# Liupeter01/Software-Rasterizer

Measured on AMD Instinct MI355X. Metric: frames_per_sec, higher is better.
Workload: dtype f32

## Files before the change

### software-rasterizer_amd/csrc/srz_api.hip

```cpp
#include <dlfcn.h>

#include <algorithm>
#include <cmath>
#include <cstdio>
#include <cstdlib>
#include <cstring>
#include <new>
#include <string>
#include <vector>

#include "srz_device.h"

using namespace srz;

namespace {
std::string g_create_error;

struct EventPair {
  hipEvent_t t0, t1, t2, t3;
  bool detailed;
};

struct BatchDesc {
  int32_t shader, tex_id;
// ... 88 lines not shown
  uint32_t *d_sparse_rows = nullptr;
  uint32_t *d_slow_list = nullptr, *d_slow_count = nullptr;
  uint4 *d_redo_list = nullptr;
  uint32_t fast_kinds = 0;
  bool any_generic = true;
  uint32_t *d_vis = nullptr, *d_work_count = nullptr, *d_chunk_rows = nullptr;
  uint4 *d_worklist = nullptr;
  uint64_t kind_slots = 0;
  uint32_t kind_mask = 0, n_kind_slots = 0;
  bool approx_shade = false;
  bool no_packed = false;
  uint32_t *d_band_desc = nullptr;
  uint2 *d_band_ent = nullptr;
  uint64_t total_groups = 0;
  ShadeDescG *d_sdesc = nullptr;
  DrawDesc *d_draws = nullptr;
  static constexpr int STAGE_RING = 4;
  uint8_t *d_dyn = nullptr;
  size_t dyn_bytes = 0, dyn_lights_off = 0, dyn_draws_off = 0;
  uint8_t *h_stage[STAGE_RING] = {};
  hipEvent_t stage_ev[STAGE_RING] = {};
  bool stage_busy[STAGE_RING] = {};
  unsigned stage_next = 0;
  std::vector<DrawDesc> h_draws;
  std::vector<int> h_draw_mesh;
  uint32_t n_draws = 0, max_faces = 0;
  uint64_t sdesc_version = 0;
  uint32_t tiles_x = 0, max_tiles = 0;
  bool have_stats = false;
  bool update_failed = false;
  static constexpr int CLEAR_TUNE_SKIP = 6, CLEAR_TUNE_AGAIN = 4096;
  struct ClearTune {
    uint32_t wgs = CLEAR_GRID_DEFAULT;
    bool done = false;
    int renders = 0;
    int since = 0;
    ClearCtl *d_ctl = nullptr;
    uint32_t *h_wgs = nullptr;
  } clear_tune;
  srz_stats stats{};
};

namespace {

hipStream_t pick_stream(const srz_ctx *ctx, void *stream) {
  if (!stream) return ctx->stream;
// ... 303 lines not shown
  if (!ct.done && ct.renders == 0)
    if (const uint32_t m = clear_memo(ctx, fs, 0u)) ct.wgs = p.wgs = m, ct.done = true;
  if (ct.done) return SRZ_OK;
  const uint32_t h = *static_cast<volatile uint32_t *>(ct.h_wgs);
  const int j = ct.renders - srz_frameset::CLEAR_TUNE_SKIP;
  if (h != 0u) {
    ct.wgs = p.wgs = h, ct.done = true;
    clear_memo(ctx, fs, h);
  } else if (!detailed && j < 0) {
    p.count = true;
  } else if (!detailed) {
    p.wgs = CLEAR_GRID_MAX, p.dev_wgs = &ct.d_ctl->wgs;
    p.count = p.stamp = j < CLEAR_TUNE_RENDERS;
  }
  return SRZ_OK;
}

void end_clear_plan(srz_frameset *fs, const ClearPlan &p, hipStream_t s) {
  if (p.count) ++fs->clear_tune.renders;
  if (p.stamp) launch_clear_tune(fs->clear_tune.d_ctl, fs->clear_tune.h_wgs, s);
  if (p.rebase) launch_clear_rebase(fs->clear_tune.d_ctl, s);
}

struct RenderPlan {
  Pass pass;
  hipStream_t s;
  bool side, turns, vertex_setup;
  ClearPlan clear;
  EventPair *ep;
};

int enqueue_sub_batch(srz_ctx *ctx, srz_frameset *fs, const RenderPlan &r, RenderArgs &a, int f0, int n, int part) {
  const bool stats = r.pass.kind == Pass::COUNTING;
  const hipStream_t s = r.s;
  const size_t tpf = (size_t)fs->n_local_bands * fs->tiles_x;
  RenderArgs v = a;
  if (n != fs->n_frames) {
    const int fa = r.pass.f_begin + f0;
    v.frames += fa, v.n_frames = (uint32_t)n;
    v.vis += (size_t)fa * tpf * ((size_t)TILE * TILE);
    v.tile_info += (size_t)fa * tpf;
    v.out += (size_t)fa * a.frame_stride;
    v.work_cap = (uint32_t)((size_t)(n < 8 ? n : (n + 7) / 8) * tpf);
  }
  const uint32_t tiles = (uint32_t)((size_t)n * tpf);
  if (r.vertex_setup) launch_chunks(v, n, fs->max_tris, s);
  else launch_setup(v, n, fs->max_tris, stats, s);
  launch_bin(v, n, fs->max_tris, s);
  if (!fs->pool_sized && !stats) {
    HIP_TRY(ctx, copy_demand(fs, part, s));
    HIP_TRY(ctx, hipStreamSynchronize(s));
    const uint32_t need = max_pool_demand(fs, part, part + 1);
    if (need > fs->pool_sub_cap) {
      if (int rc = grow_pool(ctx, fs, need, 8u)) return rc;
      a.pool = v.pool = fs->d_pool, a.pool_sub_cap = v.pool_sub_cap = fs->pool_sub_cap;
      HIP_TRY(ctx, hipMemsetAsync(fs->d_pool_heads, 0, sizeof(uint32_t) * CNT_STRIDE * fs->pool_n_sub, s));
      launch_bin(v, n, fs->max_tris, s);
    }
  }
  if (r.pass.kind == Pass::SIZE_ONLY) return SRZ_OK;
  if (r.ep) HIP_TRY(ctx, hipEventRecord(r.ep->t1, s));
  const unsigned ev = r.side ? ctx->ev_next++ % srz_ctx::EV_RING : 0u;
  if (r.side) {
    HIP_TRY(ctx, hipEventRecord(ctx->ev_fork[ev], s));
    HIP_TRY(ctx, hipStreamWaitEvent(ctx->stream2, ctx->ev_fork[ev], 0));
    launch_clear(v, tiles, ctx->stream2, r.clear.wgs);
    HIP_TRY(ctx, copy_demand(fs, part, ctx->stream2));
    HIP_TRY(ctx, hipEventRecord(ctx->ev_join[ev], ctx->stream2));
  }
// ... 26 lines not shown
  const uint32_t need = max_pool_demand(fs, 0, srz_frameset::DEMAND_PARTS);
  if (need > fs->pool_sub_cap)
    if (int rc = grow_pool(ctx, fs, need, 4u)) return rc;
  RenderArgs a = make_args(ctx, fs, d_out, flags_or, pass);
  if (!size_only) fs->last_flags = flags_or, fs->rendered = true;
  EventPair ep{};
  const bool timed = ctx->timing != 0 && !stats && !size_only && ctx->ev_used.size() < 65536, detailed = timed && ctx->timing >= 2;
  if (timed)
    if (int rc = begin_timing(ctx, ep, detailed, s)) return rc;
  if (stats) HIP_TRY(ctx, hipMemsetAsync(ctx->d_stats, 0, ST_COUNT * sizeof(unsigned long long), s));
  if (fs->max_tris == 0) {
    HIP_TRY(ctx, hipMemsetAsync(fs->d_work_count, 0, sizeof(uint32_t) * CNT_STRIDE * N_WORK_LISTS, s));
    HIP_TRY(ctx, hipMemsetAsync(fs->d_pool_heads, 0, sizeof(uint32_t) * CNT_STRIDE * fs->pool_n_sub, s));
    HIP_TRY(ctx, hipMemsetAsync(fs->d_slow_count, 0, 2 * sizeof(uint32_t), s));
  }
  const bool turns = !stats && !size_only && fs->max_tiles >= 8192;
  if (turns && !ctx->ev_raster[0])
    if (int rc = create_side(ctx, "render: raster events", nullptr, false, ctx->ev_raster)) return rc;
  if (turns && ctx->raster_valid && ctx->raster_last_stream != s) {
    HIP_TRY(ctx, hipStreamWaitEvent(s, ctx->ev_raster[(ctx->raster_next + srz_ctx::EV_RING - 1) % srz_ctx::EV_RING], 0));
    a.other_streams = 1u;
  }
  const bool vertex_setup = fs->d_draws != nullptr && !stats;
  if (fs->d_draws) launch_vertex(fs->d_draws, fs->n_draws, fs->max_faces, fs->d_tris, fs->d_tri_pos, fs->d_frames, vertex_setup ? fs->d_bbox : nullptr, s);
  const bool any_fused = any_frame_has(fs, flags_or, SRZ_FUSED_CLEAR), side = any_fused && fs->max_tiles >= 8192 && !size_only;
  if (side && !ctx->stream2)
    if (int rc = create_side(ctx, "render: clear stream", &ctx->stream2, true, ctx->ev_fork, ctx->ev_join)) return rc;
  if (!side && any_fused) a.clear_in_raster = 1u;
  RenderPlan r{pass, s, side, turns, vertex_setup, ClearPlan{}, detailed ? &ep : nullptr};
  if (side)
    if (int rc = plan_clear(ctx, fs, pass, detailed, s, r.clear)) return rc;
  a.clear_wgs_dev = r.clear.dev_wgs;
  const int n_all = pass.f_count < 0 ? fs->n_frames : pass.f_count;
  const int chunk = sub_batch_frames(ctx, fs, n_all, stats || detailed);
  for (int f0 = 0, part = 0; f0 < n_all; f0 += chunk, ++part)
    if (int rc = enqueue_sub_batch(ctx, fs, r, a, f0, std::min(chunk, n_all - f0), part)) return rc;
  if (!stats) fs->pool_sized = true;
  end_clear_plan(fs, r.clear, s);
  if (timed) {
    HIP_TRY(ctx, hipEventRecord(ep.t3, s));
    ctx->ev_used.push_back(ep);
  }
  HIP_TRY(ctx, hipGetLastError());
  return SRZ_OK;
}

int render_entry(const char *name, srz_ctx *ctx, srz_frameset *fs, void *d_out, size_t out_bytes, uint32_t flags, void *stream, Pass pass) {
  if (!ctx) return SRZ_E_INVALID;
  const std::string fn(name);
  if (!fs || !d_out) return fail(ctx, SRZ_E_INVALID, fn + ": null frameset / output");
  if (out_bytes < srz_frameset_out_bytes(ctx, fs)) return fail(ctx, SRZ_E_INVALID, fn + ": output buffer too small");
  if (((uintptr_t)d_out & 15u) != 0) return fail(ctx, SRZ_E_INVALID, fn + ": output must be 16-byte aligned");
// ... 130 lines not shown
  if (e != hipSuccess) {
    (void)hipFree(d_px);
    return fail(ctx, SRZ_E_NODEVICE, std::string("srz_texture_upload: ") + hipGetErrorString(e));
  }
  (void)hipFree(ctx->d_texmem[tex_id]);
  ctx->d_texmem[tex_id] = d_px;
  ctx->h_tex[tex_id] = TexDesc{d_px, w, h};
  ctx->tex_version++;
  return SRZ_OK;
}

static void set_shading(FrameDesc &d, const srz_frame &fr) {
  std::memcpy(d.eye, fr.eye, sizeof d.eye), std::memcpy(d.ka, fr.ka, sizeof d.ka), std::memcpy(d.ks, fr.ks, sizeof d.ks);
  d.p = fr.p, d.kh = fr.kh, d.kn = fr.kn;
  d.flags = fr.flags & FRAME_FLAGS;
}

static void stage_dyn(const srz_frameset *fs, uint8_t *st) {
  std::memcpy(st, fs->h_frames.data(), sizeof(FrameDesc) * fs->h_frames.size());
  if (!fs->h_lights.empty()) std::memcpy(st + fs->dyn_lights_off, fs->h_lights.data(), sizeof(srz_light) * fs->h_lights.size());
  if (!fs->h_draws.empty()) std::memcpy(st + fs->dyn_draws_off, fs->h_draws.data(), sizeof(DrawDesc) * fs->h_draws.size());
}

static int ensure_stage_ring(srz_ctx *ctx, srz_frameset *fs, const char *who) {
  if (fs->h_stage[0]) return SRZ_OK;
  for (int i = 0; i < srz_frameset::STAGE_RING; ++i) {
    hipError_t e = hipHostMalloc((void **)&fs->h_stage[i], fs->dyn_bytes, hipHostMallocDefault);
    if (e == hipSuccess) e = hipEventCreateWithFlags(&fs->stage_ev[i], hipEventDisableTiming);
    if (e != hipSuccess) {
      for (int j = 0; j <= i; ++j) {
        if (fs->h_stage[j]) (void)hipHostFree(fs->h_stage[j]);
        if (fs->stage_ev[j]) (void)hipEventDestroy(fs->stage_ev[j]);
        fs->h_stage[j] = nullptr, fs->stage_ev[j] = nullptr;
      }
      return fail(ctx, e == hipErrorOutOfMemory ? SRZ_E_NOMEM : SRZ_E_NODEVICE, std::string(who) + ": staging buffers: " + hipGetErrorString(e));
    }
  }
  return SRZ_OK;
}

static int upload_dyn(srz_ctx *ctx, srz_frameset *fs) {
  const unsigned slot = fs->stage_next++ % srz_frameset::STAGE_RING;
  if (fs->stage_busy[slot]) HIP_TRY(ctx, hipEventSynchronize(fs->stage_ev[slot]));
  stage_dyn(fs, fs->h_stage[slot]);
  HIP_TRY(ctx, hipMemcpyAsync(fs->d_dyn, fs->h_stage[slot], fs->dyn_bytes, hipMemcpyHostToDevice, ctx->stream));
  HIP_TRY(ctx, hipEventRecord(fs->stage_ev[slot], ctx->stream));
  fs->stage_busy[slot] = true;
  return SRZ_OK;
}

static int build_frameset(srz_ctx *ctx, const srz_frame *frames, int n_frames, srz_frameset **out, bool copy_tris, bool tris_aos = false,
                          const std::vector<DrawDesc> *draws = nullptr) {
  if (!ctx) return SRZ_E_INVALID;
  if (!out) return fail(ctx, SRZ_E_INVALID, "srz_frameset_create: out is NULL");
  *out = nullptr;
  if (!frames || n_frames <= 0) return fail(ctx, SRZ_E_INVALID, "srz_frameset_create: no frames");
  const int W = frames[0].width, H = frames[0].height;
  if (W <= 0 || H <= 0 || W > 32767 || H > 32767) return fail(ctx, SRZ_E_INVALID, "srz_frameset_create: width/height must be in 1..32767");
  HIP_TRY(ctx, hipSetDevice(ctx->device));
  srz_frameset *fs = new (std::nothrow) srz_frameset();
  if (!fs) return fail(ctx, SRZ_E_NOMEM, "srz_frameset_create: out of host memory");
  fs->n_frames = n_frames, fs->width = W, fs->height = H;
  fs->shard_rank = ctx->shard_rank, fs->shard_world = ctx->shard_world;
  shard_layout(H, fs->shard_rank, fs->shard_world, fs->n_bands, fs->n_local_bands, fs->bands_per_rank, fs->local_rows);
  fs->tiles_x = (uint32_t)((W + TILE - 1) / TILE);
  if ((uint64_t)((n_frames + 7) / 8 * 8) * fs->n_local_bands * fs->tiles_x >= 0x7fffffffull) {
    delete fs;
    return fail(ctx, SRZ_E_INVALID, "srz_frameset_create: frames x tiles exceeds the launch grid limit; split the batch");
  }
  uint64_t tri_off = 0, light_off = 0, batch_off = 0, group_off = 0;
  for (int f = 0; f < n_frames; ++f) {
    const srz_frame &fr = frames[f];
// ... 42 lines not shown
    const FrameDesc &d = fs->h_frames[f];
    size_t o = d.tri_off;
    for (uint32_t b = 0; b < fr.n_batches; ++b) {
      const srz_batch &sb = fr.batches[b];
      if (copy_tris && sb.n_tris) {
        std::memcpy(&h_tris[o], sb.tris, sizeof(srz_tri) * sb.n_tris);
        if (!h_pos.empty())
          for (size_t t = 0; t < sb.n_tris; ++t) std::memcpy(&h_pos[(o + t) * TRI_POS_F], &sb.tris[t].pos[0][0], sizeof(float) * TRI_POS_F);
      }
      std::fill(h_tb.begin() + o, h_tb.begin() + o + sb.n_tris, (uint16_t)b);
      o += sb.n_tris;
    }
    if (fr.n_lights) std::memcpy(&fs->h_lights[d.light_off], fr.lights, sizeof(srz_light) * fr.n_lights);
  }
  classify_frames(fs);
  if (draws) {
    fs->h_draws = *draws, fs->n_draws = (uint32_t)draws->size();
    for (const DrawDesc &dd : *draws) fs->max_faces = std::max(fs->max_faces, dd.n_faces);
  }
  auto up16 = [](size_t v) { return (v + 15) & ~(size_t)15; };
  fs->dyn_lights_off = up16(sizeof(FrameDesc) * (size_t)n_frames);
  fs->dyn_draws_off = up16(fs->dyn_lights_off + sizeof(srz_light) * (size_t)light_off);
  fs->dyn_bytes = fs->dyn_draws_off + sizeof(DrawDesc) * fs->h_draws.size();
  auto dev_alloc = [&](void **p, size_t bytes) { return hipMalloc(p, std::max<size_t>(bytes, 256)); };
  hipError_t e = hipSuccess;
#define FS_TRY(expr)                                                                                                   \
  if (e == hipSuccess) e = (expr)
  FS_TRY(dev_alloc((void **)&fs->d_dyn, fs->dyn_bytes));
  if (e == hipSuccess) {
    fs->d_frames = reinterpret_cast<FrameDesc *>(fs->d_dyn);
    fs->d_lights = reinterpret_cast<srz_light *>(fs->d_dyn + fs->dyn_lights_off);
    if (draws) fs->d_draws = reinterpret_cast<DrawDesc *>(fs->d_dyn + fs->dyn_draws_off);
  }
  FS_TRY(dev_alloc((void **)&fs->d_tris, sizeof(srz_tri) * tri_off));
  if (!fs->tris_aos) FS_TRY(dev_alloc((void **)&fs->d_tri_pos, sizeof(float) * TRI_POS_F * tri_off + 16));
  FS_TRY(dev_alloc((void **)&fs->d_bbox, sizeof(BBox) * tri_off));
  FS_TRY(dev_alloc((void **)&fs->d_chunk_rows, sizeof(uint32_t) * (tri_off / 64 + (size_t)n_frames + 1)));
  FS_TRY(dev_alloc((void **)&fs->d_band_desc, sizeof(uint32_t) * group_off * fs->n_local_bands));
  FS_TRY(dev_alloc((void **)&fs->d_band_ent, sizeof(uint2) * group_off * ENT_PER_GROUP));
  FS_TRY(dev_alloc((void **)&fs->d_tri_batch, sizeof(uint16_t) * tri_off));
  fs->max_tiles = (uint32_t)n_frames * fs->n_local_bands * fs->tiles_x;
  {
    const uint64_t n_wgs = (uint64_t)((n_frames + 7) / 8 * 8) * fs->n_local_bands;
    uint32_t n_sub = 1;
    while (n_sub < 64u && (uint64_t)n_sub * 256u <= n_wgs) n_sub *= 2u;
    fs->pool_n_sub = n_sub;
// ... 273 lines not shown

int srz_frameset_render(srz_ctx *ctx, srz_frameset *fs, void *d_out, size_t out_bytes, uint32_t flags, void *stream) {
  return render_entry("srz_frameset_render", ctx, fs, d_out, out_bytes, flags, stream, Pass::colour());
}

int srz_frameset_render_visibility(srz_ctx *ctx, srz_frameset *fs, void *d_out, size_t out_bytes, uint32_t flags, void *stream) {
  return render_entry("srz_frameset_render_visibility", ctx, fs, d_out, out_bytes, flags, stream, Pass::visibility());
}

int srz_frameset_shade_visibility(srz_ctx *ctx, srz_frameset *fs, const void *d_vis, void *d_out, size_t out_bytes, uint32_t flags,
                                  void *stream) {
  if (!ctx) return SRZ_E_INVALID;
  const std::string fn("srz_frameset_shade_visibility");
  if (!fs || !d_vis || !d_out) return fail(ctx, SRZ_E_INVALID, fn + ": null frameset / visibility buffer / output");
  const size_t bytes = srz_frameset_out_bytes(ctx, fs);
  if (out_bytes < bytes) return fail(ctx, SRZ_E_INVALID, fn + ": output buffer too small");
  if ((((uintptr_t)d_vis | (uintptr_t)d_out) & 15u) != 0) return fail(ctx, SRZ_E_INVALID, fn + ": buffers must be 16-byte aligned");
  const uintptr_t v = (uintptr_t)d_vis, o = (uintptr_t)d_out;
  if (v != o && v < o + bytes && o < v + bytes) return fail(ctx, SRZ_E_INVALID, fn + ": visibility buffer and output overlap partly");
  if (int rc = check_renderable(ctx, fs)) return rc;
  HIP_TRY(ctx, hipSetDevice(ctx->device));
  const hipStream_t s = pick_stream(ctx, stream);
  if (int rc = resolve_shading(ctx, fs, s)) return rc;
  if (fs->d_draws) launch_vertex(fs->d_draws, fs->n_draws, fs->max_faces, fs->d_tris, fs->d_tri_pos, fs->d_frames, nullptr, s);
  ShadeVisArgs a{};
  a.frames = fs->d_frames, a.tris = fs->d_tris, a.tri_batch = fs->d_tri_batch, a.lights = fs->d_lights, a.sdesc = fs->d_sdesc;
  a.vis = (const float *)d_vis, a.out = (float *)d_out;
  a.frame_stride = 4ull * fs->local_rows * (uint64_t)fs->width;
  a.local_rows = fs->local_rows, a.tiles_x = fs->tiles_x, a.n_local_bands = fs->n_local_bands, a.n_frames = (uint32_t)fs->n_frames;
  a.shard_rank = fs->shard_rank, a.shard_world = fs->shard_world;
  a.flags_or = flags & FRAME_FLAGS, a.in_place = v == o ? 1u : 0u;
  a.any_generic = fs->any_generic ? 1u : 0u;
  a.redo_list = reinterpret_cast<uint32_t *>(fs->d_redo_list), a.redo_count = fs->d_slow_count + 1;
  HIP_TRY(ctx, hipMemsetAsync(a.redo_count, 0, sizeof(uint32_t), s));
  launch_shade_vis(a, fs->fast_kinds, fs->any_generic, fs->approx_shade, s);
  const srz_frameset::ClearTune &ct = fs->clear_tune;
  if (!ctx->env_clear_wgs && ct.d_ctl && !ct.done && fs->max_tiles >= 8192) launch_clear_rebase(ct.d_ctl, s);
  HIP_TRY(ctx, hipGetLastError());
  return SRZ_OK;
}

int srz_frameset_update_shading(srz_ctx *ctx, srz_frameset *fs, const srz_frame *frames, int n_frames) {
  if (!ctx) return SRZ_E_INVALID;
  if (!fs || !frames) return fail(ctx, SRZ_E_INVALID, "srz_frameset_update_shading: null frameset / frames");
  if (fs->d_draws) return fail(ctx, SRZ_E_INVALID, "srz_frameset_update_shading: a sceneset (its shading changes with srz_sceneset_update)");
  HIP_TRY(ctx, hipSetDevice(ctx->device));
// ... 359 lines not shown
}
extern "C" {

size_t srz_frameset_sparse_capacity(const srz_ctx *ctx, const srz_frameset *fs, int what) {
  if (!fs || !sparse_kind(what)) return 0;
  const SparseArgs a = sparse_args(fs, what);
  return (size_t)(a.payload_off + (uint64_t)a.n_frames * a.bands_per_rank * a.tiles_x * sparse_tile_bytes(a));
}

int srz_frameset_sparse_pack(srz_ctx *ctx, srz_frameset *fs, const void *d_shard, void *d_msg, size_t msg_bytes, int what, void *stream) {
  if (!ctx) return SRZ_E_INVALID;
  if (!fs || !d_shard || !d_msg || !sparse_kind(what)) return fail(ctx, SRZ_E_INVALID, "srz_frameset_sparse_pack: bad arguments");
  if (fs->shard_rank != ctx->shard_rank || fs->shard_world != ctx->shard_world)
    return fail(ctx, SRZ_E_INVALID, "srz_frameset_sparse_pack: the frameset was created under a different shard");
  const size_t cap = srz_frameset_sparse_capacity(ctx, fs, what);
  if (msg_bytes < cap)
    return fail(ctx, SRZ_E_INVALID, "srz_frameset_sparse_pack: message buffer of " + std::to_string(msg_bytes) + " bytes, " +
                                        std::to_string(cap) + " needed (srz_frameset_sparse_capacity)");
  if ((uintptr_t)d_msg & 15u) return fail(ctx, SRZ_E_INVALID, "srz_frameset_sparse_pack: the message must be 16-byte aligned");
  if (!fs->rendered) return fail(ctx, SRZ_E_INVALID, "srz_frameset_sparse_pack: the frameset has not been rendered");
  HIP_TRY(ctx, hipSetDevice(ctx->device));
  hipStream_t s = pick_stream(ctx, stream);
  if (!fs->d_sparse_rows) HIP_TRY(ctx, hipMalloc(&fs->d_sparse_rows, sizeof(uint32_t) * std::max<size_t>((size_t)fs->n_frames * fs->bands_per_rank, 1)));
  SparseArgs a = sparse_args(fs, what);
  a.shard = d_shard, a.msg = static_cast<uint8_t *>(d_msg);
  launch_sparse_pack(a, s);
  HIP_TRY(ctx, hipGetLastError());
  return SRZ_OK;
}

int srz_frameset_sparse_unpack(srz_ctx *ctx, const srz_frameset *fs, const void *d_recv, size_t msg_stride, void *d_gathered, int what,
                               void *stream) {
  if (!ctx) return SRZ_E_INVALID;
  if (!fs || !d_recv || !d_gathered || !sparse_kind(what)) return fail(ctx, SRZ_E_INVALID, "srz_frameset_sparse_unpack: bad arguments");
  if (fs->shard_rank != ctx->shard_rank || fs->shard_world != ctx->shard_world)
    return fail(ctx, SRZ_E_INVALID, "srz_frameset_sparse_unpack: the frameset was created under a different shard");
  const SparseArgs a = sparse_args(fs, what);
  if (msg_stride < a.payload_off || (msg_stride & 15u) || ((uintptr_t)d_recv & 15u))
    return fail(ctx, SRZ_E_INVALID, "srz_frameset_sparse_unpack: the stride must be a multiple of 16 bytes of at least a message's header and "
                                    "table (" + std::to_string(a.payload_off) + " bytes), the messages 16-byte aligned");
  if (what == SRZ_EXCHANGE_PLANES && ((uintptr_t)d_gathered & 3u)) return fail(ctx, SRZ_E_INVALID, "srz_frameset_sparse_unpack: misaligned buffer");
  if (fs->shard_world == 1) return SRZ_OK;
  HIP_TRY(ctx, hipSetDevice(ctx->device));
  launch_sparse_unpack(a, d_recv, msg_stride, d_gathered, pick_stream(ctx, stream));
  HIP_TRY(ctx, hipGetLastError());
  return SRZ_OK;
// ... 64 lines not shown
int srz_sync(srz_ctx *ctx) {
  if (!ctx) return SRZ_E_INVALID;
  HIP_TRY(ctx, hipSetDevice(ctx->device));
  HIP_TRY(ctx, hipStreamSynchronize(ctx->stream));
  return SRZ_OK;
}

static int refresh_frames(srz_ctx *ctx, srz_frameset *fs, const srz_frame *frames, int n_frames, const char *who, bool copy_tris) {
  auto bad = [&](int code, const char *what) { return fail(ctx, code, std::string(who) + ": " + what); };
  if (n_frames != fs->n_frames) return bad(SRZ_E_INVALID, "frame count changed");
  for (int f = 0; f < n_frames; ++f) {
    const srz_frame &fr = frames[f];
    const FrameDesc &d = fs->h_frames[f];
    if (fr.width != fs->width || fr.height != fs->height) return bad(SRZ_E_INVALID, "frame size changed");
    if (fr.n_lights != d.n_lights || (fr.n_lights && !fr.lights)) return bad(SRZ_E_INVALID, "light count changed");
    if (fr.n_batches != d.n_batches || (fr.n_batches && !fr.batches)) return bad(SRZ_E_INVALID, "batch count changed");
    for (uint32_t b = 0; b < fr.n_batches; ++b) {
      const srz_batch &sb = fr.batches[b];
      if (sb.n_tris != fs->h_batches[d.batch_off + b].count) return bad(SRZ_E_INVALID, "triangle count of a batch changed");
      if (sb.shader < SRZ_SHADER_NORMAL || sb.shader > SRZ_SHADER_BUMP) return bad(SRZ_E_INVALID, "unknown shader type");
      if (copy_tris && sb.n_tris && !sb.tris) return bad(SRZ_E_INVALID, "batch with null triangle pointer");
    }
  }
  if (int rc = ensure_stage_ring(ctx, fs, who)) return rc;
  bool batches_changed = false;
  for (int f = 0; f < n_frames; ++f) {
    const srz_frame &fr = frames[f];
    FrameDesc &d = fs->h_frames[f];
    set_shading(d, fr);
    if (fr.n_lights) std::memcpy(&fs->h_lights[d.light_off], fr.lights, sizeof(srz_light) * fr.n_lights);
    for (uint32_t b = 0; b < fr.n_batches; ++b) {
      BatchDesc &bd = fs->h_batches[d.batch_off + b];
      if (bd.shader != fr.batches[b].shader || bd.tex_id != fr.batches[b].tex_id)
        bd.shader = fr.batches[b].shader, bd.tex_id = fr.batches[b].tex_id, batches_changed = true;
    }
  }
  classify_frames(fs);
  fs->update_failed = ensure_worklists(fs) != hipSuccess;
  if (fs->update_failed) return bad(SRZ_E_NOMEM, "hipMalloc of the work lists failed");
  if (int rc = upload_dyn(ctx, fs)) return rc;
  if (batches_changed) fs->sdesc_version = 0;
  if (copy_tris) {
    for (int f = 0; f < n_frames; ++f) {
      size_t o = fs->h_frames[f].tri_off;
      for (uint32_t b = 0; b < frames[f].n_batches; ++b) {
        const srz_batch &sb = frames[f].batches[b];
        if (sb.n_tris) HIP_TRY(ctx, hipMemcpyAsync(fs->d_tris + o, sb.tris, sizeof(srz_tri) * sb.n_tris, hipMemcpyHostToDevice, ctx->stream));
        o += sb.n_tris;
      }
    }
  }
  fs->have_stats = false;
  return SRZ_OK;
}

static int draw_impl(srz_ctx *ctx, int primitive, const srz_frame *frame, const srz_scene_frame *scene, float *z, float *c0,
                     float *c1, float *c2, srz_stats *stats) {
  if (!ctx) return SRZ_E_INVALID;
  if (primitive != SRZ_PRIMITIVE_LINES && primitive != SRZ_PRIMITIVE_TRIANGLES)
    return fail(ctx, SRZ_E_PRIMITIVE, "Primitive Type is not supported!");
  if ((!frame && !scene) || !z || !c0 || !c1 || !c2) return fail(ctx, SRZ_E_INVALID, "srz_draw: null argument");
  if (ctx->shard_world != 1) return fail(ctx, SRZ_E_INVALID, "srz_draw: whole-frame draw needs an unsharded ctx (srz_set_shard(ctx,0,1))");
  HIP_TRY(ctx, hipSetDevice(ctx->device));
// ... 134 lines not shown
```

### software-rasterizer_amd/csrc/srz_device.h

```cpp
#pragma once
#include <hip/hip_runtime.h>
#include <stdint.h>

#include "../../include/srz.h"

namespace srz {

constexpr int TILE = 32;
constexpr int BAND = 32;
constexpr int KEY_STRIDE = TILE + 1;
constexpr int LDS_STRIDE = 32;
#ifndef SRZ_BAND_ROT
#define SRZ_BAND_ROT 5
#endif
__host__ __device__ inline int band_rot(int world) { return (SRZ_BAND_ROT % world) ? SRZ_BAND_ROT : (SRZ_BAND_ROT ? 1 : 0); }
__host__ __device__ inline int band_of(int lb, int rank, int world) {
  if (world == 1) return lb;
  int j = (rank - band_rot(world) * lb) % world;
  return lb * world + (j < 0 ? j + world : j);
}
__host__ __device__ inline int rank_of_band(int b, int world) { return (b + band_rot(world) * (b / world)) % world; }
constexpr uint32_t NO_TRI = 0xffffffffu;
constexpr uint32_t CNT_STRIDE = 32;
constexpr uint32_t FD_FAST_SHADE = 0x100u, FD_NL_SHIFT = 9;
// ... 100 lines not shown
  int32_t shard_rank, shard_world;
  uint32_t flags_or;
  unsigned long long *stats;
  const uint32_t *clear_wgs_dev;
};

constexpr int CLEAR_CANDS = 3, CLEAR_TUNE_BLOCK = 3, CLEAR_TUNE_RENDERS = 2 * CLEAR_CANDS * CLEAR_TUNE_BLOCK;
constexpr uint32_t CLEAR_CAND[CLEAR_CANDS] = {96, 128, 256};
constexpr uint32_t CLEAR_GRID_MAX = 256, CLEAR_GRID_DEFAULT = 96;
struct ClearCtl {
  uint32_t wgs;
  uint32_t cur, pos, phase, done, alive;
  uint32_t n[CLEAR_CANDS];
  unsigned long long last;
  float t[CLEAR_CANDS][4];
  float score[CLEAR_CANDS];
};
void launch_clear_tune(ClearCtl *ctl, uint32_t *h_wgs, hipStream_t s);
void launch_clear_rebase(ClearCtl *ctl, hipStream_t s);

void launch_vertex(const DrawDesc *draws, uint32_t n_draws, uint32_t max_faces, srz_tri *tris, float *tri_pos, const FrameDesc *frames,
                   BBox *bbox_out, hipStream_t s);
void launch_chunks(const RenderArgs &a, int n_frames, uint32_t max_tris, hipStream_t s);
void launch_setup(const RenderArgs &a, int n_frames, uint32_t max_tris, bool stats, hipStream_t s);
void launch_bin(const RenderArgs &a, int n_frames, uint32_t max_tris, hipStream_t s);
void launch_raster(const RenderArgs &a, int n_frames, bool stats, hipStream_t s);
bool raster_four_waves(const RenderArgs &a);
void launch_clear(const RenderArgs &a, uint32_t max_tiles, hipStream_t s, uint32_t wgs);
void launch_shade(const RenderArgs &a, uint32_t max_tiles, bool stats, uint32_t kinds, bool any_generic, bool approx, hipStream_t s);
void launch_visibility(const RenderArgs &a, uint32_t max_tiles, hipStream_t s);
struct ShadeVisArgs {
  const FrameDesc *frames;
  const srz_tri *tris;
  const uint16_t *tri_batch;
  const srz_light *lights;
  const ShadeDescG *sdesc;
  const float *vis;
  float *out;
  uint64_t frame_stride;
  uint32_t local_rows, tiles_x, n_local_bands, n_frames;
  int32_t shard_rank, shard_world;
  uint32_t flags_or, in_place;
  uint32_t any_generic;
  uint32_t *redo_list;
  uint32_t *redo_count;
};
// ... 30 lines not shown
```

### software-rasterizer_amd/csrc/srz_kernels.hip

```cpp
#include "srz_device.h"

#include <algorithm>
#include <cstdio>
#include <cstdlib>
#include <type_traits>

#pragma clang fp contract(off)

namespace srz {

#define SRZ_CAS __attribute__((address_space(4)))
template <typename T> __device__ __forceinline__ const SRZ_CAS T *as_const(const T *p) { return (const SRZ_CAS T *)(p); }
typedef float f32x4 __attribute__((ext_vector_type(4)));
typedef unsigned int u32x2 __attribute__((ext_vector_type(2)));
typedef unsigned int u32x4 __attribute__((ext_vector_type(4)));

__device__ __forceinline__ float sse_max(float a, float b) { return a > b ? a : b; }
__device__ __forceinline__ float sse_min(float a, float b) { return a < b ? a : b; }
__device__ __forceinline__ float std_max(float a, float b) { return (a < b) ? b : a; }
__device__ __forceinline__ float std_clamp(float v, float lo, float hi) { return (v < lo) ? lo : (hi < v) ? hi : v; }
__device__ __forceinline__ float fmsubf(float a, float b, float c) { return __builtin_fmaf(a, b, -c); }
__device__ __forceinline__ float fmaf_(float a, float b, float c) { return __builtin_fmaf(a, b, c); }

__device__ __forceinline__ uint32_t f2u_(float f) { return __builtin_bit_cast(uint32_t, f); }
// ... 528 lines not shown
  }
}

__global__ __launch_bounds__(256) void k_chunks(RenderArgs a) {
  __shared__ uint32_t s_cnt[MAX_LOCAL_BANDS], s_off[MAX_LOCAL_BANDS], s_fill[MAX_LOCAL_BANDS], s_misc[2];
  if (blockIdx.x == 0 && blockIdx.y == 0) reset_render_counters(a);
  const SRZ_CAS FrameDesc *fd = as_const(a.frames) + blockIdx.y;
  const uint32_t n_tris = fd->n_tris, tri_off = fd->tri_off;
  const SRZ_CAS u32x2 *bbox = as_const(reinterpret_cast<const u32x2 *>(a.bbox + tri_off));
  const uint32_t n_groups = (n_tris + GROUP_TRIS - 1u) / GROUP_TRIS;
  for (uint32_t g = blockIdx.x; g < n_groups; g += gridDim.x) {
    const uint32_t t0 = g * GROUP_TRIS;
    BBox bb[GROUP_K];
    bool keep[GROUP_K];
#pragma unroll
    for (int k = 0; k < (int)GROUP_K; ++k) {
      const uint32_t t = t0 + (uint32_t)k * 256u + threadIdx.x;
      bb[k].sx = 1, bb[k].sy = 1, bb[k].ex = 0, bb[k].ey = 0;
      if (t < n_tris) {
        const u32x2 r = bbox[t];
        bb[k].sx = (int16_t)(r.x & 0xffff), bb[k].sy = (int16_t)(r.x >> 16), bb[k].ex = (int16_t)(r.y & 0xffff), bb[k].ey = (int16_t)(r.y >> 16);
      }
      keep[k] = bb[k].sx <= bb[k].ex;
      chunk_rows_store(a, fd->chunk_off, t, n_tris, keep[k], bb[k]);
    }
    bucket_group(a, fd->n_local_bands, fd->group_off + g, t0, (fd->flags & FD_PACKED) != 0u, tri_off, bb, keep, nullptr, s_cnt, s_off, s_fill, s_misc);
  }
}

constexpr int BIN_MAX_WAVES = 8;
constexpr uint32_t BIN_STAGE = 4096;
__host__ __device__ constexpr uint32_t bin_keep(uint32_t waves) { return waves >= 8u ? 4u : 1u; }
__global__ __launch_bounds__(64 * BIN_MAX_WAVES) void k_bin(RenderArgs a) {
  const int BIN_WAVES = (int)(blockDim.x >> 6);
  extern __shared__ __attribute__((aligned(16))) uint32_t s_dyn[];
  const uint32_t TX = a.tiles_x;
  uint32_t *s_cnt = s_dyn, *s_off = s_dyn + TX, *s_fill = s_dyn + 2 * TX, *s_marks = s_dyn + 3 * TX;
  uint32_t *s_misc = s_marks + 64 * BIN_WAVES;
  uint32_t *s_stage = s_misc + 4;

  const uint32_t wg = blockIdx.x, xcd = wg & 7u, jj = wg >> 3;
  const uint32_t frame = (jj / a.n_local_bands) * 8u + xcd, lb = jj % a.n_local_bands;
  if (frame >= a.n_frames) return;
  const SRZ_CAS FrameDesc *fd = as_const(a.frames) + frame;
  const int lane = threadIdx.x & 63;
  const int wave = __builtin_amdgcn_readfirstlane((int)(threadIdx.x >> 6));
// ... 2295 lines not shown
__global__ void k_tex_convert(const uint8_t *bgr, int w, int h, int row_stride, uint32_t *out) {
  int i = blockIdx.x * blockDim.x + threadIdx.x;
  if (i >= w * h) return;
  int y = i / w, x = i - y * w;
  const uint8_t *p = bgr + (size_t)y * row_stride + (size_t)x * 3;
  out[i] = (uint32_t)p[0] | ((uint32_t)p[1] << 8) | ((uint32_t)p[2] << 16);
}

void launch_vertex(const DrawDesc *draws, uint32_t n_draws, uint32_t max_faces, srz_tri *tris, float *tri_pos, const FrameDesc *frames,
                   BBox *bbox_out, hipStream_t s) {
  if (n_draws == 0 || max_faces == 0) return;
  dim3 grid((max_faces + 255) / 256, n_draws);
  if (grid.x > 1024) grid.x = 1024;
  hipLaunchKernelGGL(k_vertex, grid, dim3(256), 0, s, draws, tris, tri_pos, frames, bbox_out);
}

void launch_chunks(const RenderArgs &a, int n_frames, uint32_t max_tris, hipStream_t s) {
  if (n_frames <= 0 || max_tris == 0) return;
  dim3 grid((max_tris + GROUP_TRIS - 1u) / GROUP_TRIS, n_frames);
  if (grid.x > 4096) grid.x = 4096;
  hipLaunchKernelGGL(k_chunks, grid, dim3(256), 0, s, a);
}

void launch_setup(const RenderArgs &a, int n_frames, uint32_t max_tris, bool stats, hipStream_t s) {
  if (n_frames <= 0 || max_tris == 0) return;
  dim3 grid((max_tris + GROUP_TRIS - 1u) / GROUP_TRIS, n_frames);
  if (grid.x > 4096) grid.x = 4096;
  BBox *bb = const_cast<BBox *>(a.bbox);
  if (stats)
    hipLaunchKernelGGL(k_setup<true>, grid, dim3(256), 0, s, a, bb);
  else
    hipLaunchKernelGGL(k_setup<false>, grid, dim3(256), 0, s, a, bb);
}

void launch_bin(const RenderArgs &a, int n_frames, uint32_t max_tris, hipStream_t s) {
  if (n_frames <= 0 || a.n_local_bands == 0) return;
  const uint32_t groups = ((uint32_t)n_frames + 7u) / 8u;
  const int waves = (max_tris <= 32768u && (uint32_t)n_frames * a.n_local_bands > 256u) ? 4 : BIN_MAX_WAVES;
  const size_t lds = sizeof(uint32_t) * (3u * (size_t)a.tiles_x + 64u * waves + 4u + BIN_STAGE + 2u + 128u * waves * bin_keep((uint32_t)waves));
  hipLaunchKernelGGL(k_bin, dim3(groups * 8u * a.n_local_bands), dim3(64 * waves), lds, s, a);
}

__global__ void k_clear_tune(ClearCtl *c, uint32_t *h_wgs) {
  const unsigned long long now = __builtin_amdgcn_s_memrealtime();
  if (c->done) return;
  if (c->pos > 0 && c->n[c->cur] < 4u) c->t[c->cur][c->n[c->cur]++] = (float)(now - c->last);
// ... 137 lines not shown
```

### software-rasterizer_amd/host/include/SoftRasterizer.hpp

```cpp
#pragma once
#include <array>
#include <cstdint>
#include <memory>
#include <optional>
#include <stdexcept>
#include <string>
#include <tuple>
#include <unordered_map>
#include <utility>
#include <vector>

#include "glm_min.hpp"

struct srz_ctx;
struct srz_target;
struct srz_frameset;

namespace SoftRasterizer {

struct light_struct {
  light_struct() : position(0.f), intensity(0.f) {}
  light_struct(const glm::vec3 &pos, const glm::vec3 &intense) : position(pos), intensity(intense) {}
  glm::vec3 position;
  glm::vec3 intensity;
// ... 193 lines not shown
  bool m_justCleared = false;
  void syncToHost();
  srz_ctx *m_ctx = nullptr;
  srz_target *m_target = nullptr;
  bool m_hostStale = false;
};

class TraditionalRasterizer : public RenderingPipeline {
public:
  TraditionalRasterizer();
  TraditionalRasterizer(std::size_t width, std::size_t height);
  ~TraditionalRasterizer() override;
  void draw(Primitive type) override;

  struct Stats {
    uint64_t n_tris = 0, n_culled = 0, pixel_tests = 0, fragments = 0, shaded = 0, visible = 0, visible_textured = 0;
  };
  bool collect_stats = false;
  Stats last_stats;
  bool device_vertex_stage = true;

private:
  void init();
  std::unordered_map<const Scene *, srz_frameset *> m_sceneSets;
  std::unordered_map<const TextureLoader *, int> m_texSlots;
  struct MeshSlot {
    int slot;
    std::size_t n_faces;
    std::uint64_t hash;
  };
  std::unordered_map<const Object *, MeshSlot> m_meshSlots;
  int textureSlot(const std::shared_ptr<Shader> &sh);
  std::vector<std::weak_ptr<TextureLoader>> m_texOwners;
};

}
```

### software-rasterizer_amd/host/src/SoftRasterizer.cpp

```cpp
#include "SoftRasterizer.hpp"

#include <algorithm>
#include <cmath>
#include <cstdarg>
#include <cstdio>
#include <cstring>
#include <fstream>
#include <limits>
#include <sstream>
#include <stdexcept>

#include "../../../include/srz.h"

namespace SoftRasterizer {

namespace detail {
void load_image_bgr(const std::string &path, std::vector<uint8_t> &bgr, int &W, int &H);

static void log(const char *level, const char *fmt, ...) {
  std::fprintf(stderr, "[%s] ", level);
  va_list ap;
  va_start(ap, fmt);
  std::vfprintf(stderr, fmt, ap);
  va_end(ap);
// ... 459 lines not shown
      long r = (v == v && v > -1e9f && v < 1e9f) ? std::lrintf(v) : (v > 0 ? 255 : 0);
      m_frameBuffer8[i * 3 + c] = (uint8_t)(r < 0 ? 0 : (r > 255 ? 255 : r));
    }
}

TraditionalRasterizer::TraditionalRasterizer() : RenderingPipeline() { init(); }
TraditionalRasterizer::TraditionalRasterizer(std::size_t width, std::size_t height) : RenderingPipeline(width, height) { init(); }
void TraditionalRasterizer::init() {
  if (srz_abi_version() != SRZ_ABI_VERSION)
    throw std::runtime_error("TraditionalRasterizer: libsrz.so reports SRZ_ABI_VERSION " + std::to_string(srz_abi_version()) +
                             ", libsrz_host.so was built against " + std::to_string(SRZ_ABI_VERSION) + " — rebuild both");
  int dev = 0;
  if (const char *e = std::getenv("SRZ_DEVICE")) dev = std::atoi(e);
  int rc = srz_create(&m_ctx, dev);
  if (rc != SRZ_OK) throw std::runtime_error(std::string("TraditionalRasterizer: ") + srz_last_error(nullptr));
  rc = srz_target_create(m_ctx, (int)m_width, (int)m_height, &m_target);
  if (rc != SRZ_OK) {
    std::string msg = srz_last_error(m_ctx);
    srz_destroy(m_ctx);
    m_ctx = nullptr;
    throw std::runtime_error("TraditionalRasterizer: " + msg);
  }
  m_hostStale = false;
}
TraditionalRasterizer::~TraditionalRasterizer() {
  for (auto &kv : m_sceneSets) srz_frameset_destroy(m_ctx, kv.second);
  srz_target_destroy(m_ctx, m_target);
  srz_destroy(m_ctx);
}

int TraditionalRasterizer::textureSlot(const std::shared_ptr<Shader> &sh) {
  TextureLoader *tl = sh->getTextureObject().get();
  auto it = m_texSlots.find(tl);
  if (it == m_texSlots.end()) {
    int slot = (int)m_texSlots.size();
    if (slot >= 64) throw std::runtime_error("draw: more than 64 distinct textures");
    int rc = srz_texture_upload(m_ctx, slot, tl->bgr().data(), (int)tl->width(), (int)tl->height(), (int)tl->width() * 3);
    if (rc != SRZ_OK) throw std::runtime_error(std::string("draw: ") + srz_last_error(m_ctx));
    it = m_texSlots.emplace(tl, slot).first;
    m_texOwners.push_back(sh->getTextureObject());
  }
  return it->second;
}

void RenderingPipeline::finish() {
  if (m_ctx && srz_sync(m_ctx) != SRZ_OK) throw std::runtime_error(std::string("finish: ") + srz_last_error(m_ctx));
}

void TraditionalRasterizer::draw(Primitive type) {
// ... 142 lines not shown
```

Measured before the change: 331,200.

## Fuse dynamic upload, vertex transform and setup into one front kernel

For single-frame framesets with draws and small dynamic state, the host now passes frame, light and draw descriptors as a kernel argument instead of staging them through pinned memory and a separate copy. A new k_front kernel writes that state to device memory, runs the vertex transform, triangle setup and binning in one launch, and resets the counters. This removes a memcpy and the separate launch_vertex and setup kernels. Other paths now flush the deferred upload lazily. The host frame buffer is also pinned, which should speed up readback copies. The trade-off is a 2KB kernel argument, and a per-triangle loop over all draws inside the kernel.

Result: no change. 331,000 (-0.1%).

```diff
diff --git a/software-rasterizer_amd/csrc/srz_api.hip b/software-rasterizer_amd/csrc/srz_api.hip
--- a/software-rasterizer_amd/csrc/srz_api.hip
+++ b/software-rasterizer_amd/csrc/srz_api.hip
@@ -134,6 +134,7 @@
   hipEvent_t stage_ev[STAGE_RING] = {};
   bool stage_busy[STAGE_RING] = {};
   unsigned stage_next = 0;
+  bool front = false, dyn_pending = false;
   std::vector<DrawDesc> h_draws;
   std::vector<int> h_draw_mesh;
   uint32_t n_draws = 0, max_faces = 0;
@@ -483,10 +484,13 @@
   if (p.rebase) launch_clear_rebase(fs->clear_tune.d_ctl, s);
 }
 
+int flush_dyn(srz_ctx *ctx, srz_frameset *fs);
+void enqueue_front(srz_frameset *fs, const RenderArgs &a, hipStream_t s);
+
 struct RenderPlan {
   Pass pass;
   hipStream_t s;
-  bool side, turns, vertex_setup;
+  bool side, turns, vertex_setup, front;
   ClearPlan clear;
   EventPair *ep;
 };
@@ -505,7 +509,8 @@
     v.work_cap = (uint32_t)((size_t)(n < 8 ? n : (n + 7) / 8) * tpf);
   }
   const uint32_t tiles = (uint32_t)((size_t)n * tpf);
-  if (r.vertex_setup) launch_chunks(v, n, fs->max_tris, s);
+  if (r.front) enqueue_front(fs, v, s);
+  else if (r.vertex_setup) launch_chunks(v, n, fs->max_tris, s);
   else launch_setup(v, n, fs->max_tris, stats, s);
   launch_bin(v, n, fs->max_tris, s);
   if (!fs->pool_sized && !stats) {
@@ -578,12 +583,15 @@
     a.other_streams = 1u;
   }
   const bool vertex_setup = fs->d_draws != nullptr && !stats;
-  if (fs->d_draws) launch_vertex(fs->d_draws, fs->n_draws, fs->max_faces, fs->d_tris, fs->d_tri_pos, fs->d_frames, vertex_setup ? fs->d_bbox : nullptr, s);
+  const bool front = fs->front && vertex_setup;
+  if (!front)
+    if (int rc = flush_dyn(ctx, fs)) return rc;
+  if (fs->d_draws && !front) launch_vertex(fs->d_draws, fs->n_draws, fs->max_faces, fs->d_tris, fs->d_tri_pos, fs->d_frames, vertex_setup ? fs->d_bbox : nullptr, s);
   const bool any_fused = any_frame_has(fs, flags_or, SRZ_FUSED_CLEAR), side = any_fused && fs->max_tiles >= 8192 && !size_only;
   if (side && !ctx->stream2)
     if (int rc = create_side(ctx, "render: clear stream", &ctx->stream2, true, ctx->ev_fork, ctx->ev_join)) return rc;
   if (!side && any_fused) a.clear_in_raster = 1u;
-  RenderPlan r{pass, s, side, turns, vertex_setup, ClearPlan{}, detailed ? &ep : nullptr};
+  RenderPlan r{pass, s, side, turns, vertex_setup, front, ClearPlan{}, detailed ? &ep : nullptr};
   if (side)
     if (int rc = plan_clear(ctx, fs, pass, detailed, s, r.clear)) return rc;
   a.clear_wgs_dev = r.clear.dev_wgs;
@@ -760,6 +768,20 @@
   if (!fs->h_draws.empty()) std::memcpy(st + fs->dyn_draws_off, fs->h_draws.data(), sizeof(DrawDesc) * fs->h_draws.size());
 }
 
+}
+namespace {
+void enqueue_front(srz_frameset *fs, const RenderArgs &a, hipStream_t s) {
+  FrontDyn dyn;
+  stage_dyn(fs, reinterpret_cast<uint8_t *>(dyn.w));
+  FrontArgs fa{};
+  fa.d_dyn = reinterpret_cast<uint64_t *>(fs->d_dyn), fa.dyn_bytes = (uint32_t)fs->dyn_bytes, fa.draws_off = (uint32_t)fs->dyn_draws_off;
+  fa.n_draws = fs->n_draws, fa.tris = fs->d_tris, fa.tri_pos = fs->d_tri_pos, fa.bbox_out = fs->d_bbox;
+  launch_front(a, fa, dyn, fs->max_tris, s);
+  fs->dyn_pending = false;
+}
+}
+extern "C" {
+
 static int ensure_stage_ring(srz_ctx *ctx, srz_frameset *fs, const char *who) {
   if (fs->h_stage[0]) return SRZ_OK;
   for (int i = 0; i < srz_frameset::STAGE_RING; ++i) {
@@ -786,6 +808,18 @@
   fs->stage_busy[slot] = true;
   return SRZ_OK;
 }
+
+}
+namespace {
+int flush_dyn(srz_ctx *ctx, srz_frameset *fs) {
+  if (!fs->dyn_pending) return SRZ_OK;
+  if (int rc = ensure_stage_ring(ctx, fs, "render")) return rc;
+  if (int rc = upload_dyn(ctx, fs)) return rc;
+  fs->dyn_pending = false;
+  return SRZ_OK;
+}
+}
+extern "C" {
 
 static int build_frameset(srz_ctx *ctx, const srz_frame *frames, int n_frames, srz_frameset **out, bool copy_tris, bool tris_aos = false,
                           const std::vector<DrawDesc> *draws = nullptr) {
@@ -874,6 +908,7 @@
   fs->dyn_lights_off = up16(sizeof(FrameDesc) * (size_t)n_frames);
   fs->dyn_draws_off = up16(fs->dyn_lights_off + sizeof(srz_light) * (size_t)light_off);
   fs->dyn_bytes = fs->dyn_draws_off + sizeof(DrawDesc) * fs->h_draws.size();
+  fs->front = draws && n_frames == 1 && fs->max_tris > 0 && fs->dyn_bytes <= FRONT_DYN_MAX && fs->dyn_bytes % 8 == 0;
   auto dev_alloc = [&](void **p, size_t bytes) { return hipMalloc(p, std::max<size_t>(bytes, 256)); };
   hipError_t e = hipSuccess;
 #define FS_TRY(expr)                                                                                                   \
@@ -1193,6 +1228,7 @@
   HIP_TRY(ctx, hipSetDevice(ctx->device));
   const hipStream_t s = pick_stream(ctx, stream);
   if (int rc = resolve_shading(ctx, fs, s)) return rc;
+  if (int rc = flush_dyn(ctx, fs)) return rc;
   if (fs->d_draws) launch_vertex(fs->d_draws, fs->n_draws, fs->max_faces, fs->d_tris, fs->d_tri_pos, fs->d_frames, nullptr, s);
   ShadeVisArgs a{};
   a.frames = fs->d_frames, a.tris = fs->d_tris, a.tri_batch = fs->d_tri_batch, a.lights = fs->d_lights, a.sdesc = fs->d_sdesc;
@@ -1598,6 +1634,7 @@
   HIP_TRY(ctx, hipSetDevice(ctx->device));
   hipStream_t s = pick_stream(ctx, stream);
   if (!fs->d_sparse_rows) HIP_TRY(ctx, hipMalloc(&fs->d_sparse_rows, sizeof(uint32_t) * std::max<size_t>((size_t)fs->n_frames * fs->bands_per_rank, 1)));
+  if (int rc = flush_dyn(ctx, fs)) return rc;
   SparseArgs a = sparse_args(fs, what);
   a.shard = d_shard, a.msg = static_cast<uint8_t *>(d_msg);
   launch_sparse_pack(a, s);
@@ -1708,7 +1745,8 @@
       if (copy_tris && sb.n_tris && !sb.tris) return bad(SRZ_E_INVALID, "batch with null triangle pointer");
     }
   }
-  if (int rc = ensure_stage_ring(ctx, fs, who)) return rc;
+  if (!fs->front)
+    if (int rc = ensure_stage_ring(ctx, fs, who)) return rc;
   bool batches_changed = false;
   for (int f = 0; f < n_frames; ++f) {
     const srz_frame &fr = frames[f];
@@ -1724,7 +1762,8 @@
   classify_frames(fs);
   fs->update_failed = ensure_worklists(fs) != hipSuccess;
   if (fs->update_failed) return bad(SRZ_E_NOMEM, "hipMalloc of the work lists failed");
-  if (int rc = upload_dyn(ctx, fs)) return rc;
+  if (fs->front) fs->dyn_pending = true;
+  else if (int rc = upload_dyn(ctx, fs)) return rc;
   if (batches_changed) fs->sdesc_version = 0;
   if (copy_tris) {
     for (int f = 0; f < n_frames; ++f) {
diff --git a/software-rasterizer_amd/csrc/srz_device.h b/software-rasterizer_amd/csrc/srz_device.h
--- a/software-rasterizer_amd/csrc/srz_device.h
+++ b/software-rasterizer_amd/csrc/srz_device.h
@@ -146,6 +146,21 @@
 void launch_vertex(const DrawDesc *draws, uint32_t n_draws, uint32_t max_faces, srz_tri *tris, float *tri_pos, const FrameDesc *frames,
                    BBox *bbox_out, hipStream_t s);
 void launch_chunks(const RenderArgs &a, int n_frames, uint32_t max_tris, hipStream_t s);
+constexpr uint32_t FRONT_DYN_MAX = 2048;
+struct FrontDyn {
+  uint64_t w[FRONT_DYN_MAX / 8];
+};
+struct FrontArgs {
+  uint64_t *d_dyn;
+  uint32_t dyn_bytes;
+  uint32_t draws_off;
+  uint32_t n_draws;
+  srz_tri *tris;
+  float *tri_pos;
+  BBox *bbox_out;
+};
+void launch_front(const RenderArgs &a, const FrontArgs &fa, const FrontDyn &dyn, uint32_t n_tris, hipStream_t s);
+
 void launch_setup(const RenderArgs &a, int n_frames, uint32_t max_tris, bool stats, hipStream_t s);
 void launch_bin(const RenderArgs &a, int n_frames, uint32_t max_tris, hipStream_t s);
 void launch_raster(const RenderArgs &a, int n_frames, bool stats, hipStream_t s);
diff --git a/software-rasterizer_amd/csrc/srz_kernels.hip b/software-rasterizer_amd/csrc/srz_kernels.hip
--- a/software-rasterizer_amd/csrc/srz_kernels.hip
+++ b/software-rasterizer_amd/csrc/srz_kernels.hip
@@ -574,6 +574,63 @@
         bb[k].sx = (int16_t)(r.x & 0xffff), bb[k].sy = (int16_t)(r.x >> 16), bb[k].ex = (int16_t)(r.y & 0xffff), bb[k].ey = (int16_t)(r.y >> 16);
       }
       keep[k] = bb[k].sx <= bb[k].ex;
+      chunk_rows_store(a, fd->chunk_off, t, n_tris, keep[k], bb[k]);
+    }
+    bucket_group(a, fd->n_local_bands, fd->group_off + g, t0, (fd->flags & FD_PACKED) != 0u, tri_off, bb, keep, nullptr, s_cnt, s_off, s_fill, s_misc);
+  }
+}
+
+__device__ __forceinline__ void vertex_triangle(const SRZ_CAS DrawDesc *d, const SRZ_CAS srz_vertex *verts, const SRZ_CAS uint32_t *faces,
+                                                float zs, float zo, uint32_t f, srz_tri &t) {
+#pragma unroll
+  for (int k = 0; k < 3; ++k) {
+    const SRZ_CAS srz_vertex *v = verts + faces[3 * f + k];
+    const float px = v->pos[0], py = v->pos[1], pz = v->pos[2], nx = v->nrm[0], ny = v->nrm[1], nz = v->nrm[2];
+    float x, y, z;
+    xform_div_w(d->ndc_mvp, px, py, pz, x, y, z);
+    t.pos[k][0] = x, t.pos[k][1] = y, t.pos[k][2] = z * zs + zo;
+    xform_div_w(d->normal_m, nx, ny, nz, x, y, z);
+    t.nrm[k][0] = x, t.nrm[k][1] = y, t.nrm[k][2] = z;
+    t.uv[k][0] = v->uv[0], t.uv[k][1] = v->uv[1];
+  }
+}
+
+__global__ __launch_bounds__(256) void k_front(RenderArgs a, FrontArgs fa, FrontDyn dyn) {
+  __shared__ uint32_t s_cnt[MAX_LOCAL_BANDS], s_off[MAX_LOCAL_BANDS], s_fill[MAX_LOCAL_BANDS], s_misc[2];
+  if (blockIdx.x == 0) {
+    reset_render_counters(a);
+    for (uint32_t i = threadIdx.x; i < fa.dyn_bytes / 8u; i += 256u) fa.d_dyn[i] = dyn.w[i];
+  }
+  const SRZ_CAS FrameDesc *fd = as_const(reinterpret_cast<const FrameDesc *>(dyn.w));
+  const SRZ_CAS DrawDesc *draws = as_const(reinterpret_cast<const DrawDesc *>(dyn.w + fa.draws_off / 8u));
+  const int W = fd->width, H = fd->height;
+  const uint32_t n_tris = fd->n_tris, tri_off = fd->tri_off;
+  const float ex = fd->eye[0], ey = fd->eye[1], ez = fd->eye[2];
+  const uint32_t n_groups = (n_tris + GROUP_TRIS - 1u) / GROUP_TRIS;
+  for (uint32_t g = blockIdx.x; g < n_groups; g += gridDim.x) {
+    const uint32_t t0 = g * GROUP_TRIS;
+    BBox bb[GROUP_K];
+    bool keep[GROUP_K];
+#pragma unroll
+    for (int k = 0; k < (int)GROUP_K; ++k) {
+      const uint32_t t = t0 + (uint32_t)k * 256u + threadIdx.x;
+      bb[k].sx = 1, bb[k].sy = 1, bb[k].ex = 0, bb[k].ey = 0;
+      keep[k] = false;
+      for (uint32_t i = 0; i < fa.n_draws; ++i) {
+        const SRZ_CAS DrawDesc *d = draws + i;
+        const uint32_t f = tri_off + t - d->tri_off;
+        if (t < n_tris && f < d->n_faces) {
+          srz_tri tr;
+          vertex_triangle(d, as_const(d->verts), as_const(d->faces), d->zscale, d->zoffset, f, tr);
+          const size_t ti = (size_t)tri_off + t;
+          fa.tris[ti] = tr;
+          const float P[9] = {tr.pos[0][0], tr.pos[0][1], tr.pos[0][2], tr.pos[1][0], tr.pos[1][1], tr.pos[1][2], tr.pos[2][0], tr.pos[2][1], tr.pos[2][2]};
+          F3 *po = reinterpret_cast<F3 *>(fa.tri_pos + ti * TRI_POS_F);
+          po[0] = F3{P[0], P[1], P[2]}, po[1] = F3{P[3], P[4], P[5]}, po[2] = F3{P[6], P[7], P[8]};
+          keep[k] = setup_triangle(P, W, H, ex, ey, ez, true, bb[k]);
+          fa.bbox_out[ti] = bb[k];
+        }
+      }
       chunk_rows_store(a, fd->chunk_off, t, n_tris, keep[k], bb[k]);
     }
     bucket_group(a, fd->n_local_bands, fd->group_off + g, t0, (fd->flags & FD_PACKED) != 0u, tri_off, bb, keep, nullptr, s_cnt, s_off, s_fill, s_misc);
@@ -2915,6 +2972,11 @@
   hipLaunchKernelGGL(k_chunks, grid, dim3(256), 0, s, a);
 }
 
+void launch_front(const RenderArgs &a, const FrontArgs &fa, const FrontDyn &dyn, uint32_t n_tris, hipStream_t s) {
+  if (n_tris == 0) return;
+  hipLaunchKernelGGL(k_front, dim3((n_tris + GROUP_TRIS - 1u) / GROUP_TRIS), dim3(256), 0, s, a, fa, dyn);
+}
+
 void launch_setup(const RenderArgs &a, int n_frames, uint32_t max_tris, bool stats, hipStream_t s) {
   if (n_frames <= 0 || max_tris == 0) return;
   dim3 grid((max_tris + GROUP_TRIS - 1u) / GROUP_TRIS, n_frames);
diff --git a/software-rasterizer_amd/host/include/SoftRasterizer.hpp b/software-rasterizer_amd/host/include/SoftRasterizer.hpp
--- a/software-rasterizer_amd/host/include/SoftRasterizer.hpp
+++ b/software-rasterizer_amd/host/include/SoftRasterizer.hpp
@@ -239,6 +239,7 @@
 
 private:
   void init();
+  bool m_frame8Pinned = false;
   std::unordered_map<const Scene *, srz_frameset *> m_sceneSets;
   std::unordered_map<const TextureLoader *, int> m_texSlots;
   struct MeshSlot {
diff --git a/software-rasterizer_amd/host/src/SoftRasterizer.cpp b/software-rasterizer_amd/host/src/SoftRasterizer.cpp
--- a/software-rasterizer_amd/host/src/SoftRasterizer.cpp
+++ b/software-rasterizer_amd/host/src/SoftRasterizer.cpp
@@ -505,9 +505,11 @@
     throw std::runtime_error("TraditionalRasterizer: " + msg);
   }
   m_hostStale = false;
+  m_frame8Pinned = srz_host_register(m_ctx, m_frameBuffer8.data(), m_frameBuffer8.size()) == SRZ_OK;
 }
 TraditionalRasterizer::~TraditionalRasterizer() {
   for (auto &kv : m_sceneSets) srz_frameset_destroy(m_ctx, kv.second);
+  if (m_frame8Pinned) srz_host_unregister(m_ctx, m_frameBuffer8.data());
   srz_target_destroy(m_ctx, m_target);
   srz_destroy(m_ctx);
 }
```
